# aik2mlj/polyffusion

Measured on AMD Instinct MI355X. Metric: denoising steps/sec (8-bar prmat2c, batch 16), higher is better.
Workload: dtype bf16x3; 1 GPU; sdf_chd8bar cond generation, batch 16 per GPU, 1000-step DDPM sampler loop body (BASELINE.json configs[1]); weights: deterministic synthetic, 41.08M params; global_batch=16, parallelism=batch-shard x1

## Files before the change

### polyffusion_amd/build.py

```python
from __future__ import annotations

import os
import subprocess
import sys

HERE = os.path.dirname(os.path.abspath(__file__))
CSRC = os.path.join(HERE, "csrc")
SOURCES = ["conv_plan.hip", "conv_mfma.hip", "conv_bf16x3.hip", "conv_wino.hip", "gemm_planes_bf3.hip", "mlp_fused_bf3.hip", "attention.hip", "attention_bf3.hip", "norm_stats.hip", "small_kernels.hip", "encoders.hip", "decoders.hip", "comm.hip", "plan.hip", "unet_blocks.hip", "unet.hip", "attention_wide.hip", "ddpm_unet.hip", "autoencoder.hip", "loss.hip", "abi_ops.hip"]
LIB = os.path.join(HERE, "libpfhip.so")
VARIANTS = {"": [], "f16": ["-DPF_X3_F16"]}


def lib_path(variant: str = "") -> str:
    return os.path.join(HERE, f"libpfhip_{variant}.so" if variant else "libpfhip.so")
HIPCC = os.environ.get("HIPCC", "/opt/rocm/bin/hipcc")
FLAGS = ["--offload-arch=gfx950", "-O3", "-std=c++17", "-fPIC", "-Wall", "-Wno-unused-function"] + (["-DPF_TRACE"] if os.environ.get("PF_TRACE") else [])
EXTRA_FLAGS = {"attention_bf3.hip": ["-fno-slp-vectorize"]}


STAMP = os.path.join(CSRC, ".build_stamp.json")


def _digest(paths, extra=()) -> str:
    import hashlib
    h = hashlib.sha256()
    for p in paths:
        with open(p, "rb") as f:
            h.update(hashlib.sha256(f.read()).digest())
    for e in extra:
        h.update(str(e).encode())
        h.update(b"\0")
    return h.hexdigest()


def _read_stamp() -> dict:
    import json
    try:
        with open(STAMP) as f:
            return json.load(f)
    except (OSError, ValueError):
        return {}


def _write_stamp(st: dict) -> None:
    import json
    with open(STAMP + ".new", "w") as f:
        json.dump(st, f, indent=1, sort_keys=True)
    os.replace(STAMP + ".new", STAMP)


def build(force: bool = False, verbose: bool = True, variant: str = "") -> str:
    return build_all(force, verbose, (variant,))[0]


_SLOW_FIRST = ["conv_bf16x3.hip", "conv_wino.hip", "attention_bf3.hip", "mlp_fused_bf3.hip", "conv_mfma.hip", "gemm_planes_bf3.hip"]


def build_all(force: bool = False, verbose: bool = True, variants=("", "f16")) -> list:
    force = force or os.environ.get("PF_FORCE_BUILD", "") not in ("", "0")
    hdrs = [os.path.join(CSRC, h) for h in sorted(os.listdir(CSRC)) if h.endswith(".h")] + [os.path.join(HERE, "..", "include", "pfhip.h")]
    stamp = _read_stamp()
    objs, jobs, want = {v: [] for v in variants}, [], {}
    for variant in variants:
        sfx = f".{variant}" if variant else ""
        for src0 in SOURCES:
            s = os.path.join(CSRC, src0)
            src = src0 + sfx
            o = os.path.join(CSRC, src0.replace(".hip", sfx + ".o"))
            objs[variant].append(o)
            flags = FLAGS + EXTRA_FLAGS.get(src0, []) + VARIANTS[variant]
            want[src] = _digest([s] + hdrs, flags)
            if force or not os.path.exists(o) or stamp.get(src) != want[src]:
                cmd = [HIPCC] + flags + ["-c", s, "-o", o]
                if verbose:
                    print(" ".join(cmd), flush=True)
                jobs.append((src, cmd, variant, _SLOW_FIRST.index(src0) if src0 in _SLOW_FIRST else len(_SLOW_FIRST)))
    jobs.sort(key=lambda j: j[3])
    if jobs:
        from concurrent.futures import ThreadPoolExecutor
        with ThreadPoolExecutor(max_workers=min(len(jobs), os.cpu_count() or 1)) as ex:
            rcs = list(ex.map(lambda j: subprocess.run(j[1]).returncode, jobs))
        for (src, _, _, _), rc in zip(jobs, rcs):
            if rc == 0:
                stamp[src] = want[src]
            else:
                stamp.pop(src, None)
        _write_stamp(stamp)
        if any(rcs):
            raise subprocess.CalledProcessError(max(rcs), "hipcc")
    elif verbose:
        print(f"polyffusion_amd.build: {len(SOURCES)} objects per variant current by content digest (PF_FORCE_BUILD=1 recompiles)", flush=True)
    libs = []
    for variant in variants:
        lib, lib_key = lib_path(variant), os.path.basename(lib_path(variant))
        lib_want = _digest(objs[variant])
        if force or any(j[2] == variant for j in jobs) or not os.path.exists(lib) or stamp.get(lib_key) != lib_want:
            cmd = [HIPCC, "--offload-arch=gfx950", "-shared", "-fPIC", "-o", lib] + objs[variant] + ["-ldl"]
            if verbose:
                print(" ".join(cmd), flush=True)
            subprocess.check_call(cmd)
            stamp[lib_key] = lib_want
            _write_stamp(stamp)
        libs.append(lib)
    return libs


if __name__ == "__main__":
    vs = ("", "f16") if "--all" in sys.argv else tuple(a.split("=", 1)[1] for a in sys.argv if a.startswith("--variant=")) or ("",)
    build_all(force="--force" in sys.argv, variants=vs)
```

### polyffusion_amd/csrc/conv_wino.hip

```cpp
#include "conv_plan.h"

namespace pf {

typedef x3_t x3x4 __attribute__((ext_vector_type(4)));

#ifdef PF_TRACE
__device__ unsigned long long g_wtrace[3 * 256];
#define WTR() do { if (trace_on && tslot < 255) { g_wtrace[tbase + tslot++] = __builtin_amdgcn_s_memtime(); } } while (0)
#define WTR_DECL() const bool trace_on = (threadIdx.x == 0) && (blockIdx.x == 0 || blockIdx.x == gridDim.x / 2 || blockIdx.x == gridDim.x - 1); \
                   const int tbase = blockIdx.x == 0 ? 0 : (blockIdx.x == gridDim.x - 1 ? 512 : 256); int tslot = 0; (void)tbase
#else
#define WTR() do {} while (0)
#define WTR_DECL() do {} while (0)
#endif

constexpr int WPP = 36, WRP = 18 * WPP + 8, WHALO = 18 * WRP;
constexpr int WINO_LDS = 4 * 2 * 4 * 16 * 64 * 4;

__device__ __forceinline__ void lds_barrier() {
  asm volatile("s_waitcnt lgkmcnt(0)" ::: "memory");
  __builtin_amdgcn_s_barrier();
  asm volatile("" ::: "memory");
}

template <class T>
__device__ __forceinline__ const T* uniform_ptr(const T* q) {
  const unsigned long long v = reinterpret_cast<unsigned long long>(q);
  const unsigned lo = __builtin_amdgcn_readfirstlane((unsigned)v), hi = __builtin_amdgcn_readfirstlane((unsigned)(v >> 32));
  return reinterpret_cast<const T*>(((unsigned long long)hi << 32) | lo);
}

__device__ __forceinline__ __amdgpu_buffer_rsrc_t rsrc_or_empty(const void* q) {
  return __builtin_amdgcn_make_buffer_rsrc(const_cast<void*>(q), 0, q ? 0x7fffffff : 0, 0x00020000);
}
__device__ __forceinline__ const float* sbias_row_scalar(const ConvP& p, int b) {
  if (!p.sbias) return nullptr;
  long long r = b;
  if (p.sb_rows) {
    typedef const long long __attribute__((address_space(4))) * cptr;
    r = *((cptr)(unsigned long long)(p.sb_rows + b));
    r = r < 0 ? 0 : (r >= p.sb_nrows ? p.sb_nrows - 1 : r);
  }
  return p.sbias + (size_t)r * p.ld_sbias;
}

__device__ __forceinline__ void wino_epilogue(const ConvP& p, f32x16 (&acc)[4][2][2], unsigned char* smem_all, int b, int oy0, int ox0, int n0,
                                              int ty_t, int tx_t, int wave, int lane, int tid, const float* sb, bool trace_on = false, int tbase = 0, int tslot = 0) {
  (void)trace_on; (void)tbase; (void)tslot;
  const int fh = wave >> 1, fnb = wave & 1;
  const int c8 = lane & 7, tl = lane >> 3;
  const int n = n0 + fnb * 32 + c8 * 4;
  const int pix0 = (b * p.Hout + oy0 + 8 * fh) * p.Wout + ox0 + 2 * tl;
  auto pix = [&](int u, int pp, int q) { return pix0 + (2 * u + pp) * p.Wout + q; };
  const __amdgpu_buffer_rsrc_t rsRes = rsrc_or_empty(uniform_ptr(p.res)), rsOut = rsrc_or_empty(uniform_ptr(p.out));
  f32x4 rr[4][2][2];
#pragma unroll
  for (int u = 0; u < 4; ++u)
#pragma unroll
    for (int pp = 0; pp < 2; ++pp)
#pragma unroll
      for (int q = 0; q < 2; ++q)
        rr[u][pp][q] = __builtin_bit_cast(f32x4, __builtin_amdgcn_raw_buffer_load_b128(rsRes, (pix(u, pp, q) * p.ld_res + n) * 4, 0, 0));
  const f32x4 cba = __builtin_bit_cast(f32x4, __builtin_amdgcn_raw_buffer_load_b128(rsrc_or_empty(uniform_ptr(p.bias)), n * 4, 0, 0));
  const f32x4 cbb = __builtin_bit_cast(f32x4, __builtin_amdgcn_raw_buffer_load_b128(rsrc_or_empty(uniform_ptr(sb)), n * 4, 0, 0));
  const f32x4 cbc = __builtin_bit_cast(f32x4, __builtin_amdgcn_raw_buffer_load_b128(rsrc_or_empty(uniform_ptr(p.bias2)), n * 4, 0, 0));
  lds_barrier();
  float* X = reinterpret_cast<float*>(smem_all);
#pragma unroll
  for (int h = 0; h < 2; ++h)
#pragma unroll
    for (int nb = 0; nb < 2; ++nb) {
      const int blk = h * 2 + nb;
#pragma unroll
      for (int r = 0; r < 16; ++r) {
        const float s0 = acc[0][h][nb][r] + acc[1][h][nb][r] + acc[2][h][nb][r];
        const float s1 = acc[1][h][nb][r] - acc[2][h][nb][r] - acc[3][h][nb][r];
        X[((((wave * 2 + 0) * 4 + blk) * 16 + r) * 64) + lane] = s0;
        X[((((wave * 2 + 1) * 4 + blk) * 16 + r) * 64) + lane] = s1;
      }
      __builtin_amdgcn_sched_barrier(0);
    }
  WTR();
  lds_barrier();
  WTR();
  const f32x4 cb4 = cba + cbb + cbc;
  f32x4 s1 = {0.f, 0.f, 0.f, 0.f}, s2 = s1;
  unsigned am = 0;
  const float* Xr = X + (tl & 3) * 64 + ((tl >> 2) & 1) * 32 + c8 * 4;
#pragma unroll
  for (int u = 0; u < 4; ++u)
#pragma unroll
    for (int q = 0; q < 2; ++q) {
      f32x4 sv[4];
#pragma unroll
      for (int i = 0; i < 4; ++i) sv[i] = *reinterpret_cast<const f32x4*>(Xr + ((((i * 2 + q) * 4 + wave) * 16 + 4 * u) * 64));
#pragma unroll
      for (int pp = 0; pp < 2; ++pp) {
        f32x4 v = pp == 0 ? sv[0] + sv[1] + sv[2] : sv[1] - sv[2] - sv[3];
        v = PF_X3_UNSCALE(v) + cb4 + rr[u][pp][q];
        __builtin_amdgcn_raw_buffer_store_b128(__builtin_bit_cast(u32x4, v), rsOut, (pix(u, pp, q) * p.ld_out + n) * 4, 0, 0);
        if (p.amax) amax_acc4(am, v);
        s1 += v; s2 += v * v;
      }
    }
  WTR();
  amax_flush(p.amax, am);
  if (p.stats) {
    lds_barrier();
    float* red = reinterpret_cast<float*>(smem_all);
    *reinterpret_cast<f32x4*>(red + (wave * 64 + lane) * 8) = s1;
    *reinterpret_cast<f32x4*>(red + (wave * 64 + lane) * 8 + 4) = s2;
    lds_barrier();
    if (tid < 64) {
      const int nb = tid >> 5, cc = (tid & 31) >> 2, e = tid & 3;
      float a0 = 0.f, a1 = 0.f;
#pragma unroll
      for (int h = 0; h < 2; ++h)
#pragma unroll
        for (int t8 = 0; t8 < 8; ++t8) {
          const float* q = red + ((h * 2 + nb) * 64 + t8 * 8 + cc) * 8 + e;
          a0 += q[0]; a1 += q[4];
        }
      const int tile = ty_t * p.tiles_x + tx_t;
      float* dst = p.stats + (((size_t)b * (p.tiles_x * p.tiles_y) + tile) * p.N + n0 + tid) * 2;
      dst[0] = a0; dst[1] = a1;
    }
  }
  WTR();
}

typedef float f32x2_ __attribute__((ext_vector_type(2)));
__device__ __forceinline__ f32x2_ silu2(f32x2_ v) {
  f32x2_ t = v * -1.44269504088896340736f;
  t[0] = __builtin_amdgcn_exp2f(t[0]); t[1] = __builtin_amdgcn_exp2f(t[1]);
  t = t + 1.0f;
  t[0] = __builtin_amdgcn_rcpf(t[0]); t[1] = __builtin_amdgcn_rcpf(t[1]);
  return v * t;
}

__device__ __forceinline__ f32x2_ pk_sub(f32x2_ a, f32x2_ b) { f32x2_ d; asm("v_pk_add_f32 %0, %1, %2 neg_lo:[0,1] neg_hi:[0,1]" : "=v"(d) : "v"(a), "v"(b)); return d; }
__device__ __forceinline__ f32x2_ pk_fma(f32x2_ a, f32x2_ b, f32x2_ c) { f32x2_ d; asm("v_pk_fma_f32 %0, %1, %2, %3" : "=v"(d) : "v"(a), "v"(b), "v"(c)); return d; }
__device__ __forceinline__ f32x4 sub4(f32x4 a, f32x4 b) {
  const f32x2_ l = pk_sub(f32x2_{a[0], a[1]}, f32x2_{b[0], b[1]}), h = pk_sub(f32x2_{a[2], a[3]}, f32x2_{b[2], b[3]});
  return f32x4{l[0], l[1], h[0], h[1]};
}
__device__ __forceinline__ f32x4 fma4(f32x4 a, f32x2_ s2, f32x4 c) {
  const f32x2_ l = pk_fma(f32x2_{a[0], a[1]}, s2, f32x2_{c[0], c[1]}), h = pk_fma(f32x2_{a[2], a[3]}, s2, f32x2_{c[2], c[3]});
  return f32x4{l[0], l[1], h[0], h[1]};
}

typedef x3_t x3x2 __attribute__((ext_vector_type(2)));
typedef float f32x2 __attribute__((ext_vector_type(2)));
struct SplitK { unsigned c0, c1; };
__device__ __forceinline__ SplitK split_consts() {
#ifdef PF_X3_F16
  SplitK k{0x0000BC00u, 0xBC000000u};
#else
  SplitK k{0x0000BF80u, 0xBF800000u};
#endif
  asm volatile("" : "+s"(k.c0), "+s"(k.c1));
  return k;
}
__device__ __forceinline__ float x3_sub_hi(x3x2 hp, unsigned c, float v) {
#ifdef PF_X3_F16
  return __builtin_amdgcn_fdot2(hp, __builtin_bit_cast(x3x2, c), v, false);
#else
  return __builtin_amdgcn_fdot2_f32_bf16(hp, __builtin_bit_cast(x3x2, c), v, false);
#endif
}
__device__ __forceinline__ void split4(f32x4 v, x3x4& hi, x3x4& lo, SplitK k) {
  const x3x2 h01 = __builtin_convertvector(f32x2{v[0], v[1]}, x3x2), h23 = __builtin_convertvector(f32x2{v[2], v[3]}, x3x2);
  const float l0 = x3_sub_hi(h01, k.c0, v[0]), l1 = x3_sub_hi(h01, k.c1, v[1]), l2 = x3_sub_hi(h23, k.c0, v[2]), l3 = x3_sub_hi(h23, k.c1, v[3]);
  const x3x2 q01 = __builtin_convertvector(f32x2{l0, l1}, x3x2), q23 = __builtin_convertvector(f32x2{l2, l3}, x3x2);
  hi = __builtin_shufflevector(h01, h23, 0, 1, 2, 3);
  lo = __builtin_shufflevector(q01, q23, 0, 1, 2, 3);
}

template <int DUMMY>
__global__ __launch_bounds__(256, 1) void conv_wino_pipe_kernel(ConvP p) {
  extern __shared__ __attribute__((aligned(16))) unsigned char smem_all[];
  WTR_DECL();
  WTR();
  constexpr int WIMG = WHALO + 1024;
  float* H0 = reinterpret_cast<float*>(smem_all) + 1024;
  const int tid = threadIdx.x, lane = tid & 63;
  const int wave = __builtin_amdgcn_readfirstlane(tid >> 6);

  int lid;
  {
    const int nwg = gridDim.x, orig = blockIdx.x;
    const int xcd = orig & 7, q = nwg >> 3, r = nwg & 7;
    lid = __builtin_amdgcn_readfirstlane((xcd < r ? xcd * (q + 1) : r * (q + 1) + (xcd - r) * q) + (orig >> 3));
  }
  int mt = __builtin_amdgcn_readfirstlane(fdiv(lid, p.d_nt));
  const int nti = lid - mt * p.nt;
  int t = __builtin_amdgcn_readfirstlane(fdiv(mt, p.d_tx));
  const int tx_t = mt - t * p.tiles_x; mt = t;
  const int b = __builtin_amdgcn_readfirstlane(fdiv(mt, p.d_ty));
  const int ty_t = mt - b * p.tiles_y;
  const int n0 = nti * 64, oy0 = ty_t * 16, ox0 = tx_t * 16;
  conv_shared_x1(p, b);
  const int cin = p.c0 + p.c1, nchunk = cin / 32, KK = cin / 16;
  const float* sbp = sbias_row_scalar(p, b);

  if (p.gn_s0) gn_fused_prologue<256>(p, b, tid, p.Hin * p.Win, reinterpret_cast<double*>(smem_all));

  const int sub = tid & 7;
  int* gpL = reinterpret_cast<int*>(H0 + WIMG + WHALO) + tid;
  int gpr[11];
  const int bpix = b * p.Hin * p.Win;
#pragma unroll
  for (int it = 0; it < 11; ++it) {
    const int pix = min((tid >> 3) + 32 * it, 323);
    const int row = (int)__umul24(pix, 57) >> 10, col = pix - (int)__umul24(row, 18);
    const int iy = oy0 - 1 + row, ix = ox0 - 1 + col;
    const bool inside = (unsigned)iy < (unsigned)p.Hin && (unsigned)ix < (unsigned)p.Win;
    const int gpix = inside ? (int)__umul24(iy, p.Win) + ix + 1 : 0;
    const int real4 = (int)__umul24(row, WRP / 4) + (int)__umul24(col, WPP / 4) + (sub ^ ((row >> 1) & 1));
    const int lo4 = inside ? 256 + real4 : tid;
    if (!inside) {
      *reinterpret_cast<f32x4*>(H0 + real4 * 4) = f32x4{0.f, 0.f, 0.f, 0.f};
      *reinterpret_cast<f32x4*>(H0 + WIMG + real4 * 4) = f32x4{0.f, 0.f, 0.f, 0.f};
    }
    gpr[it] = gpix | (lo4 << 20);
    gpL[it * 256] = gpr[it];
  }
  const __amdgpu_buffer_rsrc_t rsSc = dma_resource(uniform_ptr(p.sc + (size_t)b * cin)), rsSh = dma_resource(uniform_ptr(p.sh + (size_t)b * cin));
  float* scL = reinterpret_cast<float*>(gpL - tid + 11 * 256);
  float* shL = scL + cin;
  const float* px0 = uniform_ptr(p.x0);
  const float* px1 = uniform_ptr(p.x1);
  f32x4 ra[11], vsc, vsh;
  auto scRead = [&](int ct) {
    vsc = *reinterpret_cast<const f32x4*>(scL + ct * 32 + sub * 4);
    vsh = *reinterpret_cast<const f32x4*>(shL + ct * 32 + sub * 4);
  };
  int gq = 0, gst = 0;
  auto gpRead = [&](int pi) { gq = gpL[pi * 256]; };
  auto haloFetch = [&](int ct, int gpv, int skip = 0) -> f32x4 {
    const int cg = ct * 32;
    const bool first = cg < p.c0;
    const __amdgpu_buffer_rsrc_t rs = dma_resource(first ? px0 : px1);
    const int cs4 = (first ? p.c0 : p.c1) * 4, co4 = (first ? cg : cg - p.c0) * 4 + bpix * cs4;
    const int gpix = (gpv & 0xFFFFF) - 1;
    const int vo = ((int)__umul24(gpix, cs4) + sub * 16) | (gpix & (int)0x80000000u) | skip;
    return __builtin_bit_cast(f32x4, __builtin_amdgcn_raw_buffer_load_b128(rs, vo, co4, 0));
  };
  auto haloLoad = [&](int pi, int ct, int gpv, int skip = 0) { ra[pi] = haloFetch(ct, gpv, skip); };
  auto stageWhole = [&](f32x4 r, f32x4 sc4, f32x4 sh4, int gpv, float* Ht) {
    r = r * sc4 + sh4;
    const f32x2_ a = silu2(f32x2_{r[0], r[1]}), c2 = silu2(f32x2_{r[2], r[3]});
    *reinterpret_cast<f32x4*>(Ht - 1024 + (((unsigned)gpv >> 20) << 2)) = f32x4{a[0], a[1], c2[0], c2[1]};
  };
  auto scLoad = [&](int ct) {
    vsc = __builtin_bit_cast(f32x4, __builtin_amdgcn_raw_buffer_load_b128(rsSc, sub * 16, ct * 128, 0));
    vsh = __builtin_bit_cast(f32x4, __builtin_amdgcn_raw_buffer_load_b128(rsSh, sub * 16, ct * 128, 0));
  };
  auto stageA = [&](int pi) {
    gst = gpL[pi * 256];
    const f32x2_ a = silu2(f32x2_{ra[pi][0], ra[pi][1]} * f32x2_{vsc[0], vsc[1]} + f32x2_{vsh[0], vsh[1]});
    ra[pi][0] = a[0]; ra[pi][1] = a[1];
  };
  auto stageB = [&](int pi, float* Ht) {
    const f32x2_ a = silu2(f32x2_{ra[pi][2], ra[pi][3]} * f32x2_{vsc[2], vsc[3]} + f32x2_{vsh[2], vsh[3]});
    ra[pi][2] = a[0]; ra[pi][3] = a[1];
    *reinterpret_cast<f32x4*>(Ht - 1024 + (((unsigned)gst >> 20) << 2)) = ra[pi];
  };

  const int m = lane & 31, g = lane >> 5, tyl = m >> 3, txl = m & 7;
  const int ax = wave == 0 ? 0 : (wave == 2 ? 2 : 1);
  const int ay = wave == 0 ? 2 : (wave == 1 ? 2 : (wave == 2 ? 1 : 3));
  const float sigma = wave == 1 ? 1.f : -1.f;
  int ox_, oy_;
  {
    const int rx = 2 * tyl + ax, ry = 2 * tyl + ay;
    ox_ = rx * WRP + (2 * txl) * WPP + (((2 * g) ^ ((rx >> 1) & 1)) << 2);
    oy_ = ry * WRP + (2 * txl) * WPP + (((2 * g) ^ ((ry >> 1) & 1)) << 2);
    asm volatile("" : "+v"(ox_), "+v"(oy_));
  }
  const SplitK spk = split_consts();
  f32x2_ sig2 = {sigma, sigma};
  asm volatile("" : "+v"(sig2));
  f32x4 rwx[2], rwy[2], tt[4];
  x3x4 fh_[2][4][2], fl_[2][4][2];
  auto fragRead = [&](const float* Hn, int s, int h, int e, int b2) {
    int ex = ox_, ey = oy_;
    if (e) { asm volatile("v_xor_b32 %0, 4, %1" : "=v"(ex) : "v"(ox_)); asm volatile("v_xor_b32 %0, 4, %1" : "=v"(ey) : "v"(oy_)); }
#pragma unroll
    for (int bb = 0; bb < 2; ++bb) {
      rwx[bb] = *reinterpret_cast<const f32x4*>(Hn + ex + ((2 * b2 + bb) * WPP + s * 16 + h * 8 * WRP));
      rwy[bb] = *reinterpret_cast<const f32x4*>(Hn + ey + ((2 * b2 + bb) * WPP + s * 16 + h * 8 * WRP));
    }
  };
  auto fragT = [&](int b2) {
#pragma unroll
    for (int bb = 0; bb < 2; ++bb) tt[2 * b2 + bb] = fma4(rwy[bb], sig2, rwx[bb]);
  };
  auto fragV = [&](int set, int j, int e) {
    const f32x4 v = j == 0 ? sub4(tt[0], tt[2]) : (j == 1 ? tt[1] + tt[2] : (j == 2 ? sub4(tt[2], tt[1]) : sub4(tt[1], tt[3])));
    split4(v, fh_[set][j][e], fl_[set][j][e], spk);
  };

  const __amdgpu_buffer_rsrc_t rsW = dma_resource(uniform_ptr(static_cast<const x3_t*>(p.w) + ((size_t)wave * KK * p.nt + nti) * 8192));
  const int wstep = p.nt * 16384;
  x3x8 bh[4][2], bl[4][2];
  auto wLoad = [&](int j, int kk) {
#pragma unroll
    for (int nb = 0; nb < 2; ++nb) {
      bh[j][nb] = __builtin_bit_cast(x3x8, __builtin_amdgcn_raw_buffer_load_b128(rsW, lane * 16, kk * wstep + ((j * 2 + nb) * 2 + 0) * 1024, 0));
      bl[j][nb] = __builtin_bit_cast(x3x8, __builtin_amdgcn_raw_buffer_load_b128(rsW, lane * 16, kk * wstep + ((j * 2 + nb) * 2 + 1) * 1024, 0));
    }
  };

  auto wLoad1 = [&](int j, int nb, bool lo, int kk, int skip) {
    if (lo) bl[j][nb] = __builtin_bit_cast(x3x8, __builtin_amdgcn_raw_buffer_load_b128(rsW, (lane * 16) | skip, kk * wstep + ((j * 2 + nb) * 2 + 1) * 1024, 0));
    else bh[j][nb] = __builtin_bit_cast(x3x8, __builtin_amdgcn_raw_buffer_load_b128(rsW, (lane * 16) | skip, kk * wstep + ((j * 2 + nb) * 2 + 0) * 1024, 0));
  };
  f32x16 acc[4][2][2];

#define SB() __builtin_amdgcn_sched_barrier(0)
  {
    const int c1 = min(1, nchunk - 1);
#pragma unroll
    for (int pi = 0; pi < 11; ++pi) haloLoad(pi, 0, gpr[pi]);
    scLoad(0);
    const f32x4 vsc0 = vsc, vsh0 = vsh;
    f32x4 rb[3];
#pragma unroll
    for (int pi = 0; pi < 3; ++pi) rb[pi] = haloFetch(c1, gpr[pi]);
    scLoad(c1);
#pragma unroll
    for (int j = 0; j < 4; ++j) wLoad(j, 0);
    float tsc[4], tsh[4];
#pragma unroll
    for (int i = 0; i < 4; ++i) {
      const int c = min(tid + 256 * i, cin - 1);
      tsc[i] = p.sc[(size_t)b * cin + c]; tsh[i] = p.sh[(size_t)b * cin + c];
    }
    WTR();
    SB();
    {
      x3x8 z8;
#pragma unroll
      for (int e = 0; e < 8; ++e) z8[e] = (x3_t)0.f;
      asm volatile("" : "+v"(z8));
      const f32x16 z16 = {0.f, 0.f, 0.f, 0.f, 0.f, 0.f, 0.f, 0.f, 0.f, 0.f, 0.f, 0.f, 0.f, 0.f, 0.f, 0.f};
#pragma unroll
      for (int j = 0; j < 4; ++j)
#pragma unroll
        for (int h = 0; h < 2; ++h)
#pragma unroll
          for (int nb = 0; nb < 2; ++nb) {
            asm volatile("" : "+v"(z8));
            acc[j][h][nb] = x3_mfma_32x32x16(z8, z8, z16, 0, 0, 0);
          }
    }
#pragma unroll
    for (int i = 0; i < 4; ++i)
      if (tid + 256 * i < cin) { scL[tid + 256 * i] = tsc[i]; shL[tid + 256 * i] = tsh[i]; }
    SB();
#pragma unroll
    for (int pi = 0; pi < 11; ++pi) stageWhole(ra[pi], vsc0, vsh0, gpr[pi], H0);
    WTR();
#pragma unroll
    for (int pi = 0; pi < 3; ++pi) stageWhole(rb[pi], vsc, vsh, gpr[pi], H0 + WIMG);
#pragma unroll
    for (int pi = 3; pi < 9; ++pi) haloLoad(pi, c1, gpr[pi]);
    WTR();
    __syncthreads();
    WTR();
#pragma unroll
    for (int e = 0; e < 2; ++e) {
      fragRead(H0, 0, 0, e, 0); fragT(0); fragRead(H0, 0, 0, e, 1); fragT(1);
#pragma unroll
      for (int j = 0; j < 4; ++j) fragV(0, j, e);
    }
  }

  for (int chunk = 0; chunk < nchunk; ++chunk) {
    const int c1 = min(chunk + 1, nchunk - 1), c2 = min(chunk + 2, nchunk - 1);
    const int skip1 = chunk + 1 < nchunk ? 0 : (int)0x80000000u, skip2 = chunk + 2 < nchunk ? 0 : (int)0x80000000u;
    float* Hcur = H0 + (chunk & 1) * WIMG;
    float* Hnxt = H0 + ((chunk + 1) & 1) * WIMG;
    static_for<0, 4>([&](auto qc) {
      constexpr int QS = decltype(qc)::value, s = QS >> 1, h = QS & 1;
      constexpr int QN = (QS + 1) & 3, sn = QN >> 1, hn = QN & 1;
      const float* Hn = QS == 3 ? Hnxt : Hcur;
      float* Ht = QS == 3 ? Hcur : Hnxt;
      constexpr int sp0 = QS == 3 ? 0 : 3 * QS + 3, spn = QS == 2 ? 2 : 3;
      constexpr int lp0 = QS == 0 ? 9 : 3 * (QS - 1), lpn = QS == 0 ? 2 : 3;
      const int lct = QS == 0 ? c1 : c2;
      WTR();
      if constexpr (QS == 3) {
        asm volatile("s_waitcnt lgkmcnt(0)" ::: "memory");
        __builtin_amdgcn_s_barrier();
        asm volatile("" ::: "memory");
      }
      SB();
      static_for<0, 24>([&](auto kc) {
        constexpr int k = decltype(kc)::value, j = k / 6, kind = (k % 6) >> 1, nb = k & 1;
        const x3x8 ah = __builtin_shufflevector(fh_[h][j][0], fh_[h][j][1], 0, 1, 2, 3, 4, 5, 6, 7);
        const x3x8 al = __builtin_shufflevector(fl_[h][j][0], fl_[h][j][1], 0, 1, 2, 3, 4, 5, 6, 7);
        if constexpr (kind == 0) acc[j][h][nb] = x3_mfma_32x32x16(al, bh[j][nb], acc[j][h][nb], 0, 0, 0);
        else if constexpr (kind == 1) acc[j][h][nb] = x3_mfma_32x32x16(ah, bl[j][nb], acc[j][h][nb], 0, 0, 0);
        else acc[j][h][nb] = x3_mfma_32x32x16(ah, bh[j][nb], acc[j][h][nb], 0, 0, 0);
        SB();
        if constexpr (k == 0 || k == 8) fragRead(Hn, sn, hn, k / 8, 0);
        if constexpr (k == 2 || k == 10) { fragT(0); fragRead(Hn, sn, hn, k / 8, 1); }
        if constexpr (k == 4 || k == 12) { fragT(1); fragV(hn, 0, k / 8); }
        if constexpr (k == 5 || k == 6 || k == 7) fragV(hn, k - 4, 0);
        if constexpr (k == 13 || k == 14 || k == 15) fragV(hn, k - 12, 1);
        if constexpr (k >= 16 && k < 16 + 2 * spn) {
          constexpr int pi = sp0 + (k - 16) / 2;
          if constexpr (((k - 16) & 1) == 0) stageA(pi); else stageB(pi, Ht);
        }
        if constexpr (k == 3 || k == 9 || k == 11) {
          constexpr int li = k == 3 ? 0 : (k == 9 ? 1 : 2);
          if constexpr (li < lpn) haloLoad(lp0 + li, lct, gq, QS == 0 ? skip1 : skip2);
        }
        if constexpr (k == 1 || k == 7 || k == 9) {
          constexpr int li = k == 1 ? 0 : (k == 7 ? 1 : 2);
          if constexpr (li < lpn) gpRead(lp0 + li);
        }
        if constexpr (k == 15) scRead(QS == 3 ? c2 : c1);
        if constexpr (h == 1 && (k % 6) >= 2) wLoad1(j, k & 1, (k % 6) < 4, s == 0 ? chunk * 2 + 1 : c1 * 2, s == 0 ? 0 : skip1);
        SB();
      });
    });
  }
#undef SB
  WTR();
#ifdef PF_TRACE
  wino_epilogue(p, acc, smem_all, b, oy0, ox0, n0, ty_t, tx_t, wave, lane, tid, sbp, trace_on, tbase, tslot);
#else
  wino_epilogue(p, acc, smem_all, b, oy0, ox0, n0, ty_t, tx_t, wave, lane, tid, sbp);
#endif
}

int launch_conv_wino(ConvP& p, const ConvPlan&, hipStream_t stream) {
  const int grid = p.B * p.tiles_y * p.tiles_x * p.nt;
  auto kern = conv_wino_pipe_kernel<0>;
  static std::atomic<uint64_t> attr_done{0};
  if (int rc = set_max_lds_once(reinterpret_cast<const void*>(kern), WINO_LDS, attr_done)) return rc;
  hipLaunchKernelGGL(kern, dim3(grid), dim3(256), WINO_LDS, stream, p);
  PF_CHECK_HIP(hipGetLastError());
  return PF_OK;
}

#ifdef PF_TRACE
extern "C" int pf_debug_wino_trace_read(unsigned long long* dst, int n) {
  return hipMemcpyFromSymbol(dst, HIP_SYMBOL(g_wtrace), (size_t)n * 8) == hipSuccess ? 0 : -1;
}
extern "C" int pf_debug_wino_trace_clear() {
  static unsigned long long z[3 * 256];
  return hipMemcpyToSymbol(HIP_SYMBOL(g_wtrace), z, sizeof z) == hipSuccess ? 0 : -1;
}
#endif

bool pack_wino_bf3(void* dst_, const float* src, int N, int K) {
  unsigned short* dst = (unsigned short*)dst_;
  bool fits = true;
  const int KK = K / 16, NT = N / 64;
  static const double G[4][3] = {{1.0, 0.0, 0.0}, {0.5, 0.5, 0.5}, {0.5, -0.5, 0.5}, {0.0, 0.0, 1.0}};
  for (int n = 0; n < N; ++n)
    for (int k = 0; k < K; ++k) {
      const float* g = src + ((size_t)n * K + k) * 9;
      double Gg[4][3];
      for (int i = 0; i < 4; ++i)
        for (int c = 0; c < 3; ++c) Gg[i][c] = G[i][0] * g[0 * 3 + c] + G[i][1] * g[1 * 3 + c] + G[i][2] * g[2 * 3 + c];
      for (int i = 0; i < 4; ++i)
        for (int j = 0; j < 4; ++j) {
          const double ud = Gg[i][0] * G[j][0] + Gg[i][1] * G[j][1] + Gg[i][2] * G[j][2];
          unsigned short hi, lo;
          fits = split_hi_lo((float)ud, &hi, &lo) && fits;
          const int kk = k / 16, ln = ((k % 16) / 8) * 32 + (n % 32), e = k % 8, ntile = n / 64, nb = (n % 64) / 32;
          const size_t frag = ((((size_t)i * KK + kk) * NT + ntile) * 4 + j) * 2 + nb;
          dst[((frag * 2 + 0) * 64 + ln) * 8 + e] = hi;
          dst[((frag * 2 + 1) * 64 + ln) * 8 + e] = lo;
        }
    }
  return fits;
}

}
```

Baseline: 211.5 steps/s.

## Cut register pressure and address math in Winograd conv pipeline kernel

```diff
diff --git a/polyffusion_amd/build.py b/polyffusion_amd/build.py
--- a/polyffusion_amd/build.py
+++ b/polyffusion_amd/build.py
@@ -15,7 +15,7 @@
     return os.path.join(HERE, f"libpfhip_{variant}.so" if variant else "libpfhip.so")
 HIPCC = os.environ.get("HIPCC", "/opt/rocm/bin/hipcc")
 FLAGS = ["--offload-arch=gfx950", "-O3", "-std=c++17", "-fPIC", "-Wall", "-Wno-unused-function"] + (["-DPF_TRACE"] if os.environ.get("PF_TRACE") else [])
-EXTRA_FLAGS = {"attention_bf3.hip": ["-fno-slp-vectorize"]}
+EXTRA_FLAGS = {"attention_bf3.hip": ["-fno-slp-vectorize"], "conv_wino.hip": ["-fno-slp-vectorize"]}
 
 
 STAMP = os.path.join(CSRC, ".build_stamp.json")
diff --git a/polyffusion_amd/csrc/conv_wino.hip b/polyffusion_amd/csrc/conv_wino.hip
--- a/polyffusion_amd/csrc/conv_wino.hip
+++ b/polyffusion_amd/csrc/conv_wino.hip
@@ -45,8 +45,11 @@
 }
 
 __device__ __forceinline__ void wino_epilogue(const ConvP& p, f32x16 (&acc)[4][2][2], unsigned char* smem_all, int b, int oy0, int ox0, int n0,
-                                              int ty_t, int tx_t, int wave, int lane, int tid, const float* sb, bool trace_on = false, int tbase = 0, int tslot = 0) {
+                                              int ty_t, int tx_t, int wave, const float* sb, bool trace_on = false, int tbase = 0, int tslot = 0) {
   (void)trace_on; (void)tbase; (void)tslot;
+  int lane;
+  asm volatile("v_mbcnt_lo_u32_b32 %0, -1, 0\n\tv_mbcnt_hi_u32_b32 %0, -1, %0" : "=v"(lane));
+  const int tid = wave * 64 + lane;
   const int fh = wave >> 1, fnb = wave & 1;
   const int c8 = lane & 7, tl = lane >> 3;
   const int n = n0 + fnb * 32 + c8 * 4;
@@ -104,7 +107,11 @@
       }
     }
   WTR();
-  amax_flush(p.amax, am);
+  if (p.amax) {
+#pragma unroll
+    for (int o = 32; o >= 1; o >>= 1) am = max(am, (unsigned)__builtin_amdgcn_ds_bpermute((lane ^ o) << 2, (int)am));
+    if (lane == 0 && am) atomicMax(p.amax, am);
+  }
   if (p.stats) {
     lds_barrier();
     float* red = reinterpret_cast<float*>(smem_all);
@@ -138,15 +145,9 @@
   return v * t;
 }
 
-__device__ __forceinline__ f32x2_ pk_sub(f32x2_ a, f32x2_ b) { f32x2_ d; asm("v_pk_add_f32 %0, %1, %2 neg_lo:[0,1] neg_hi:[0,1]" : "=v"(d) : "v"(a), "v"(b)); return d; }
-__device__ __forceinline__ f32x2_ pk_fma(f32x2_ a, f32x2_ b, f32x2_ c) { f32x2_ d; asm("v_pk_fma_f32 %0, %1, %2, %3" : "=v"(d) : "v"(a), "v"(b), "v"(c)); return d; }
-__device__ __forceinline__ f32x4 sub4(f32x4 a, f32x4 b) {
-  const f32x2_ l = pk_sub(f32x2_{a[0], a[1]}, f32x2_{b[0], b[1]}), h = pk_sub(f32x2_{a[2], a[3]}, f32x2_{b[2], b[3]});
-  return f32x4{l[0], l[1], h[0], h[1]};
-}
+__device__ __forceinline__ f32x4 sub4(f32x4 a, f32x4 b) { return f32x4{a[0] - b[0], a[1] - b[1], a[2] - b[2], a[3] - b[3]}; }
 __device__ __forceinline__ f32x4 fma4(f32x4 a, f32x2_ s2, f32x4 c) {
-  const f32x2_ l = pk_fma(f32x2_{a[0], a[1]}, s2, f32x2_{c[0], c[1]}), h = pk_fma(f32x2_{a[2], a[3]}, s2, f32x2_{c[2], c[3]});
-  return f32x4{l[0], l[1], h[0], h[1]};
+  return f32x4{__builtin_fmaf(a[0], s2[0], c[0]), __builtin_fmaf(a[1], s2[0], c[1]), __builtin_fmaf(a[2], s2[0], c[2]), __builtin_fmaf(a[3], s2[0], c[3])};
 }
 
 typedef x3_t x3x2 __attribute__((ext_vector_type(2)));
@@ -256,15 +257,28 @@
     vsc = __builtin_bit_cast(f32x4, __builtin_amdgcn_raw_buffer_load_b128(rsSc, sub * 16, ct * 128, 0));
     vsh = __builtin_bit_cast(f32x4, __builtin_amdgcn_raw_buffer_load_b128(rsSh, sub * 16, ct * 128, 0));
   };
+  f32x4 stt;
   auto stageA = [&](int pi) {
     gst = gpL[pi * 256];
-    const f32x2_ a = silu2(f32x2_{ra[pi][0], ra[pi][1]} * f32x2_{vsc[0], vsc[1]} + f32x2_{vsh[0], vsh[1]});
-    ra[pi][0] = a[0]; ra[pi][1] = a[1];
+    f32x4 v, t;
+#pragma unroll
+    for (int i = 0; i < 4; ++i) v[i] = __builtin_fmaf(ra[pi][i], vsc[i], vsh[i]);
+#pragma unroll
+    for (int i = 0; i < 4; ++i) t[i] = v[i] * -1.44269504088896340736f;
+#pragma unroll
+    for (int i = 0; i < 4; ++i) t[i] = __builtin_amdgcn_exp2f(t[i]);
+#pragma unroll
+    for (int i = 0; i < 4; ++i) t[i] = t[i] + 1.0f;
+    ra[pi] = v;
+    stt = t;
   };
   auto stageB = [&](int pi, float* Ht) {
-    const f32x2_ a = silu2(f32x2_{ra[pi][2], ra[pi][3]} * f32x2_{vsc[2], vsc[3]} + f32x2_{vsh[2], vsh[3]});
-    ra[pi][2] = a[0]; ra[pi][3] = a[1];
-    *reinterpret_cast<f32x4*>(Ht - 1024 + (((unsigned)gst >> 20) << 2)) = ra[pi];
+    f32x4 t, v;
+#pragma unroll
+    for (int i = 0; i < 4; ++i) t[i] = __builtin_amdgcn_rcpf(stt[i]);
+#pragma unroll
+    for (int i = 0; i < 4; ++i) v[i] = ra[pi][i] * t[i];
+    *reinterpret_cast<f32x4*>(Ht - 1024 + (((unsigned)gst >> 20) << 2)) = v;
   };
 
   const int m = lane & 31, g = lane >> 5, tyl = m >> 3, txl = m & 7;
@@ -283,13 +297,18 @@
   asm volatile("" : "+v"(sig2));
   f32x4 rwx[2], rwy[2], tt[4];
   x3x4 fh_[2][4][2], fl_[2][4][2];
-  auto fragRead = [&](const float* Hn, int s, int h, int e, int b2) {
-    int ex = ox_, ey = oy_;
-    if (e) { asm volatile("v_xor_b32 %0, 4, %1" : "=v"(ex) : "v"(ox_)); asm volatile("v_xor_b32 %0, 4, %1" : "=v"(ey) : "v"(oy_)); }
+  static_assert((WIMG * 4) % 32 == 0 && (1024 * 4) % 32 == 0, "the halo images start at multiples of 32 bytes");
+  typedef const f32x4 __attribute__((address_space(3)))* lds_f4;
+  int fax = (int)(unsigned)(size_t)(__attribute__((address_space(3))) float*)H0 + ox_ * 4;
+  int fay = (int)(unsigned)(size_t)(__attribute__((address_space(3))) float*)H0 + oy_ * 4;
+  asm volatile("" : "+v"(fax), "+v"(fay));
+  auto fragFlip = [&]() { asm volatile("v_xor_b32 %0, 16, %0" : "+v"(fax)); asm volatile("v_xor_b32 %0, 16, %0" : "+v"(fay)); };
+  auto fragImage = [&](int dbytes) { asm volatile("v_add_u32 %0, %1, %0" : "+v"(fax) : "s"(dbytes)); asm volatile("v_add_u32 %0, %1, %0" : "+v"(fay) : "s"(dbytes)); };
+  auto fragRead = [&](int s, int h, int b2) {
 #pragma unroll
     for (int bb = 0; bb < 2; ++bb) {
-      rwx[bb] = *reinterpret_cast<const f32x4*>(Hn + ex + ((2 * b2 + bb) * WPP + s * 16 + h * 8 * WRP));
-      rwy[bb] = *reinterpret_cast<const f32x4*>(Hn + ey + ((2 * b2 + bb) * WPP + s * 16 + h * 8 * WRP));
+      rwx[bb] = *reinterpret_cast<lds_f4>(fax + ((2 * b2 + bb) * WPP + s * 16 + h * 8 * WRP) * 4);
+      rwy[bb] = *reinterpret_cast<lds_f4>(fay + ((2 * b2 + bb) * WPP + s * 16 + h * 8 * WRP) * 4);
     }
   };
   auto fragT = [&](int b2) {
@@ -371,9 +390,10 @@
     WTR();
 #pragma unroll
     for (int e = 0; e < 2; ++e) {
-      fragRead(H0, 0, 0, e, 0); fragT(0); fragRead(H0, 0, 0, e, 1); fragT(1);
+      fragRead(0, 0, 0); fragT(0); fragRead(0, 0, 1); fragT(1);
 #pragma unroll
       for (int j = 0; j < 4; ++j) fragV(0, j, e);
+      fragFlip();
     }
   }
 
@@ -382,10 +402,10 @@
     const int skip1 = chunk + 1 < nchunk ? 0 : (int)0x80000000u, skip2 = chunk + 2 < nchunk ? 0 : (int)0x80000000u;
     float* Hcur = H0 + (chunk & 1) * WIMG;
     float* Hnxt = H0 + ((chunk + 1) & 1) * WIMG;
+    const int imgd = (chunk & 1) ? -WIMG * 4 : WIMG * 4;
     static_for<0, 4>([&](auto qc) {
       constexpr int QS = decltype(qc)::value, s = QS >> 1, h = QS & 1;
       constexpr int QN = (QS + 1) & 3, sn = QN >> 1, hn = QN & 1;
-      const float* Hn = QS == 3 ? Hnxt : Hcur;
       float* Ht = QS == 3 ? Hcur : Hnxt;
       constexpr int sp0 = QS == 3 ? 0 : 3 * QS + 3, spn = QS == 2 ? 2 : 3;
       constexpr int lp0 = QS == 0 ? 9 : 3 * (QS - 1), lpn = QS == 0 ? 2 : 3;
@@ -405,8 +425,10 @@
         else if constexpr (kind == 1) acc[j][h][nb] = x3_mfma_32x32x16(ah, bl[j][nb], acc[j][h][nb], 0, 0, 0);
         else acc[j][h][nb] = x3_mfma_32x32x16(ah, bh[j][nb], acc[j][h][nb], 0, 0, 0);
         SB();
-        if constexpr (k == 0 || k == 8) fragRead(Hn, sn, hn, k / 8, 0);
-        if constexpr (k == 2 || k == 10) { fragT(0); fragRead(Hn, sn, hn, k / 8, 1); }
+        if constexpr (k == 8) fragFlip();
+        if constexpr (k == 0 || k == 8) fragRead(sn, hn, 0);
+        if constexpr (k == 2 || k == 10) { fragT(0); fragRead(sn, hn, 1); }
+        if constexpr (k == 11) { fragFlip(); if constexpr (QS == 2) fragImage(imgd); }
         if constexpr (k == 4 || k == 12) { fragT(1); fragV(hn, 0, k / 8); }
         if constexpr (k == 5 || k == 6 || k == 7) fragV(hn, k - 4, 0);
         if constexpr (k == 13 || k == 14 || k == 15) fragV(hn, k - 12, 1);
@@ -422,7 +444,7 @@
           constexpr int li = k == 1 ? 0 : (k == 7 ? 1 : 2);
           if constexpr (li < lpn) gpRead(lp0 + li);
         }
-        if constexpr (k == 15) scRead(QS == 3 ? c2 : c1);
+        if constexpr (k == 13) scRead(QS == 3 ? c2 : c1);
         if constexpr (h == 1 && (k % 6) >= 2) wLoad1(j, k & 1, (k % 6) < 4, s == 0 ? chunk * 2 + 1 : c1 * 2, s == 0 ? 0 : skip1);
         SB();
       });
@@ -431,9 +453,9 @@
 #undef SB
   WTR();
 #ifdef PF_TRACE
-  wino_epilogue(p, acc, smem_all, b, oy0, ox0, n0, ty_t, tx_t, wave, lane, tid, sbp, trace_on, tbase, tslot);
+  wino_epilogue(p, acc, smem_all, b, oy0, ox0, n0, ty_t, tx_t, wave, sbp, trace_on, tbase, tslot);
 #else
-  wino_epilogue(p, acc, smem_all, b, oy0, ox0, n0, ty_t, tx_t, wave, lane, tid, sbp);
+  wino_epilogue(p, acc, smem_all, b, oy0, ox0, n0, ty_t, tx_t, wave, sbp);
 #endif
 }
 
```

Measured after the change: 212.5 steps/s (median of 6 runs). About the same (+0.5%).
